# BichenWuUCB/squeezeDet

Measured on NVIDIA H100. Metric: images/sec (1242x375, b=20), higher is better.
Workload: dtype f32 (3xTF32 wgmma, fp32 accumulate)

## Files before the change

include/sqdet_b200.h:

```cpp
#ifndef SQDET_B200_H_
#define SQDET_B200_H_

#include <stdint.h>

#ifdef __cplusplus
extern "C" {
#endif

#define SQDET_OK                 0
#define SQDET_ERR_INVALID_ARG   (-1)
#define SQDET_ERR_CUDA          (-2)
#define SQDET_ERR_UNSUPPORTED   (-3)
#define SQDET_ERR_STATE         (-4)
#define SQDET_ERR_NOT_FOUND     (-5)
#define SQDET_ERR_OVERFLOW      (-6)

#define SQDET_PAD_SAME   0
#define SQDET_PAD_VALID  1

#define SQDET_MATH_FP32_SIMT   0
#define SQDET_MATH_TF32X3_TC   1

typedef struct sqdet_engine sqdet_engine;

// ... 96 lines not shown
                         const int32_t* crops, int order, int rescale, void* stream);
int sqdet_forward_tiles(sqdet_engine* e, int n, int format, const uint8_t* const* planes,
                        const int64_t* pitches, const int32_t* heights, const int32_t* widths,
                        int t, const int32_t* tiles, int order, void* stream);
int sqdet_tile_results_dev(sqdet_engine* e, sqdet_det** dets, int32_t** counts,
                           int32_t* max_dets);
int sqdet_set_box_scale(sqdet_engine* e, const float* xy_scales);
int sqdet_launches_per_forward(sqdet_engine* e);
void* sqdet_engine_stream(sqdet_engine* e);

int sqdet_comm_unique_id(void* id128);
int sqdet_comm_init(sqdet_engine* e, int nranks, int rank, const void* id128);
int sqdet_comm_attach(sqdet_engine* e, void* nccl_comm, int nranks, int rank);
int sqdet_comm_destroy(sqdet_engine* e);
int sqdet_set_gather_in_forward(sqdet_engine* e, int on);
int sqdet_allgather(sqdet_engine* e, void* nccl_comm, void* stream);
int sqdet_gathered_dev(sqdet_engine* e, void** gathered_dev, int64_t* bytes_per_rank,
                       int32_t* nranks);

int sqdet_conv2d(const float* x_dev, const float* w_hwio_dev, const float* bias_dev,
                 const float* scale_dev, const float* shift_dev, float* y_dev,
                 int B, int H, int W, int Cin, int Cout, int size, int stride,
                 int padding, int relu, int y_cstride, int y_coff, int math_mode,
                 void* stream);
int sqdet_conv2d_k_split(const float* x_dev, const float* w_hwio_dev, const float* bias_dev,
                         const float* scale_dev, const float* shift_dev, float* y_dev,
                         int B, int H, int W, int Cin, int Cout, int size, int stride,
                         int padding, int relu, int y_cstride, int y_coff, int math_mode,
                         int k_split, void* stream);
int sqdet_fire(const float* x_dev, const float* w_sq_dev, const float* b_sq_dev,
               const float* w_e1_dev, const float* b_e1_dev, const float* w_e3_dev,
               const float* b_e3_dev, float* y_dev, int B, int H, int W, int Cin, int S,
               int E1, int E3, int math_mode, void* stream);
int sqdet_maxpool_nhwc(const float* x_dev, float* y_dev, int B, int H, int W, int C,
                       int size, int stride, int padding, void* stream);
#define SQDET_PRE_RESIZE_THEN_SUB 0
#define SQDET_PRE_SUB_THEN_RESIZE 1
int sqdet_preprocess_u8(const uint8_t* src_dev, int src_h, int src_w, float* dst_dev,
                        int dst_h, int dst_w, const double* bgr_means, int order,
                        void* stream);
int sqdet_interpret(const float* preds_dev, const float* anchors_f32_dev,
                    float* det_boxes_dev, float* det_probs_dev, int64_t* det_class_dev,
                    int B, int grid_h, int grid_w, int anchors_per_grid, int classes,
                    int image_width, int image_height, float exp_thresh, void* stream);
int sqdet_topk_nms(const float* boxes_dev, const float* probs_dev,
                   const int64_t* cls_dev, int B, int A, int classes, int top_n,
                   float prob_thresh, float nms_thresh, sqdet_det* dets_dev,
                   int32_t* counts_dev, int max_dets, void* stream);
int sqdet_merge_tiles(const float* boxes_dev, const float* probs_dev, const int64_t* cls_dev,
                      int A, int t, const int32_t* tile_frames, const int32_t* tile_xy, int n,
                      int classes, int top_n, float prob_thresh, float nms_thresh,
                      sqdet_det* dets_dev, int32_t* counts_dev, int max_dets, void* stream);
typedef struct sqdet_draw_style {
  int32_t            classes;
  const char* const* class_names;
  const uint8_t*     class_bgr;
  float              plot_prob_thresh;
  float              font_scale;
} sqdet_draw_style;
int sqdet_draw_dets(int n, int format, uint8_t* const* planes, const int64_t* pitches,
                    const int32_t* heights, const int32_t* widths, const int32_t* crops,
                    const sqdet_det* dets_dev, const int32_t* counts_dev, int max_dets,
                    const sqdet_draw_style* style, void* stream);

int64_t sqdet_jpeg_max_bytes(int h, int w);
int64_t sqdet_jpeg_scratch_bytes(int n, const int32_t* heights, const int32_t* widths,
// ... 101 lines not shown
```

squeezedet_b200/_lib.py:

```python
from __future__ import annotations

import ctypes as C
import os

import numpy as np

_HERE = os.path.dirname(os.path.abspath(__file__))
LIB_PATH = os.path.join(_HERE, 'lib', 'libsqdet_b200.so')

OK = 0
PAD_SAME, PAD_VALID = 0, 1
MATH_FP32_SIMT, MATH_TF32X3_TC = 0, 1
IMG_F32, IMG_U8 = 0, 1
_PAD = {'SAME': PAD_SAME, 'VALID': PAD_VALID}


class SqdetError(RuntimeError):
  def __init__(self, code, msg):
    super().__init__('sqdet error %d: %s' % (code, msg))
    self.code = code


class Det(C.Structure):
  _fields_ = [('anchor', C.c_int32), ('cls', C.c_int32), ('prob', C.c_float),
              ('cx', C.c_float), ('cy', C.c_float), ('w', C.c_float),
              ('h', C.c_float)]


DET_DTYPE = np.dtype([('anchor', '<i4'), ('cls', '<i4'), ('prob', '<f4'),
                      ('cx', '<f4'), ('cy', '<f4'), ('w', '<f4'), ('h', '<f4')])
assert DET_DTYPE.itemsize == C.sizeof(Det) == 28


class Config(C.Structure):
  _fields_ = [('batch_size', C.c_int32), ('image_height', C.c_int32),
              ('image_width', C.c_int32), ('classes', C.c_int32),
              ('anchors_per_grid', C.c_int32), ('top_n_detection', C.c_int32),
              ('prob_thresh', C.c_float), ('nms_thresh', C.c_float),
              ('exp_thresh', C.c_float), ('batch_norm_epsilon', C.c_float),
              ('math_mode', C.c_int32), ('max_dets', C.c_int32)]


class DrawStyle(C.Structure):
  _fields_ = [('classes', C.c_int32), ('class_names', C.POINTER(C.c_char_p)),
              ('class_bgr', C.POINTER(C.c_uint8)), ('plot_prob_thresh', C.c_float),
# ... 33 lines not shown
    'sqdet_read_tensor': (_i, [_vp, _i, _fp]),
    'sqdet_num_ops': (_i, [_vp]),
    'sqdet_op_info': (_i, [_vp, _i, C.c_char_p, _i, _i64p, _i64p, _i64p]),
    'sqdet_op_k_split': (_i, [_vp, _i]),
    'sqdet_forward': (_i, [_vp, _fp, _vp]),
    'sqdet_forward_n': (_i, [_vp, _fp, _i, _vp]),
    'sqdet_forward_u8': (_i, [_vp, _vp, _i, _vp]),
    'sqdet_forward_profiled': (_i, [_vp, _fp, _vp, _fp]),
    'sqdet_results_dev': (_i, [_vp, C.POINTER(_vp), C.POINTER(_vp), C.POINTER(_vp),
                               C.POINTER(_vp), C.POINTER(_vp), C.POINTER(C.c_int32)]),
    'sqdet_detect': (_i, [_vp, _fp, _fp, _fp, _fp, _fp, _fp, _vp]),
    'sqdet_set_bgr_means': (_i, [_vp, _vp]),
    'sqdet_submit': (_i, [_vp, _vp, _i, _vp, _vp]),
    'sqdet_wait': (_i, [_vp]),
    'sqdet_submit_frames': (_i, [_vp, _vp, _vp, _vp, _i, _i, _vp, _vp]),
    'sqdet_submit_frames_n': (_i, [_vp, _i, _vp, _vp, _vp, _i, _i, _vp, _vp]),
    'sqdet_forward_frames_u8': (_i, [_vp, _i, _vp, _vp, _vp, _vp, _i, _i, _vp]),
    'sqdet_forward_frames_nv12': (_i, [_vp, _i, _vp, _vp, _vp, _vp, _vp, _vp, _vp, _i, _i, _vp]),
    'sqdet_forward_frames': (_i, [_vp, _i, _i, _vp, _vp, _vp, _vp, _vp, _i, _i, _vp]),
    'sqdet_forward_tiles': (_i, [_vp, _i, _i, _vp, _vp, _vp, _vp, _i, _vp, _i, _vp]),
    'sqdet_tile_results_dev': (_i, [_vp, C.POINTER(_vp), C.POINTER(_vp), C.POINTER(C.c_int32)]),
    'sqdet_set_box_scale': (_i, [_vp, _vp]),
    'sqdet_launches_per_forward': (_i, [_vp]),
    'sqdet_engine_stream': (_vp, [_vp]),
    'sqdet_comm_unique_id': (_i, [_vp]),
    'sqdet_comm_init': (_i, [_vp, _i, _i, _vp]),
    'sqdet_comm_attach': (_i, [_vp, _vp, _i, _i]),
    'sqdet_comm_destroy': (_i, [_vp]),
    'sqdet_set_gather_in_forward': (_i, [_vp, _i]),
    'sqdet_allgather': (_i, [_vp, _vp, _vp]),
    'sqdet_gathered_dev': (_i, [_vp, C.POINTER(_vp), C.POINTER(C.c_int64),
                                C.POINTER(C.c_int32)]),
    'sqdet_fire': (_i, [_fp] * 8 + [_i] * 8 + [_vp]),
    'sqdet_conv2d': (_i, [_fp, _fp, _fp, _fp, _fp, _fp] + [_i] * 12 + [_vp]),
    'sqdet_conv2d_k_split': (_i, [_fp, _fp, _fp, _fp, _fp, _fp] + [_i] * 13 + [_vp]),
    'sqdet_maxpool_nhwc': (_i, [_fp, _fp] + [_i] * 7 + [_vp]),
    'sqdet_preprocess_u8': (_i, [_vp, _i, _i, _fp, _i, _i, _vp, _i, _vp]),
    'sqdet_interpret': (_i, [_fp, _fp, _fp, _fp, _fp] + [_i] * 7 + [_f, _vp]),
    'sqdet_topk_nms': (_i, [_fp, _fp, _fp, _i, _i, _i, _i, _f, _f, _fp, _fp, _i, _vp]),
    'sqdet_merge_tiles': (_i, [_fp, _fp, _fp, _i, _i, _vp, _vp, _i, _i, _i, _f, _f, _fp, _fp, _i,
                               _vp]),
    'sqdet_draw_dets': (_i, [_i, _i, _vp, _vp, _vp, _vp, _vp, _vp, _vp, _i, C.POINTER(DrawStyle),
                             _vp]),
    'sqdet_jpeg_max_bytes': (_i64, [_i, _i]),
    'sqdet_jpeg_scratch_bytes': (_i64, [_i, _vp, _vp, _vp]),
    'sqdet_encode_jpeg': (_i, [_i, _i, _vp, _vp, _vp, _vp, _vp, _i, _vp, _i64, _vp, _vp, _i64, _vp]),
    'sqdet_png_max_bytes': (_i64, [_i, _i]),
    'sqdet_png_scratch_bytes': (_i64, [_i, _vp, _vp, _vp]),
    'sqdet_encode_png': (_i, [_i, _i, _vp, _vp, _vp, _vp, _vp, _vp, _i64, _vp, _vp, _i64, _vp]),
    'sqdet_kitti_eval_scratch_bytes': (_i64, [_i, _i, _i64]),
    'sqdet_kitti_eval': (_i, [_i, _i, _vp, _vp, _i, _vp, _vp, _vp, _i64, _vp, _i64, _vp, _vp]),
    'sqdet_jpeg_parse': (_i, [_vp, _i64, C.POINTER(JpegInfo)]),
    'sqdet_jpeg_decode_staging_bytes': (_i64, [_i, _vp, _vp]),
    'sqdet_jpeg_decode_scratch_bytes': (_i64, [_i, _vp, _vp]),
    'sqdet_decode_jpeg': (_i, [_i, _vp, _vp, _vp, _vp, _vp, _i64, _vp, _i64, _vp, _vp]),
    'sqdet_jpeg_decode_set_subsequence_bits': (_i, [_i]),
    'sqdet_malloc': (_i, [_i, _i64, C.POINTER(_vp)]),
    'sqdet_free': (_i, [_i, _vp]),
    'sqdet_malloc_host': (_i, [_i64, C.POINTER(_vp)]),
    'sqdet_free_host': (_i, [_vp]),
    'sqdet_memcpy_h2d': (_i, [_vp, _vp, _i64, _vp]),
    'sqdet_memcpy_d2h': (_i, [_vp, _vp, _i64, _vp]),
    'sqdet_stream_sync': (_i, [_i, _vp]),
}

_lib = None
# ... 138 lines not shown
```

squeezedet_b200/csrc/conv_tc.cu:

```cuda
#include <cuda.h>
#include <cuda_runtime.h>
#include <stdint.h>
#include <stdlib.h>
#include <string.h>

#include <vector>

#include "common.cuh"
#include "conv_tc.cuh"

namespace sqdet {
namespace {

constexpr int TILE_M = 128;
constexpr int NUM_THREADS = 256;
constexpr int STAGES = 3;
constexpr int MAX_CHUNKS = 32;
constexpr int FT_W = 16, FQ_W = FT_W + 2, FQ_P = 10 * FQ_W;

enum TcMode { TC_ROWS, TC_GATHER, TC_HALO, TC_FIRE };

struct TcChunk {
  int ksize, pad_t, pad_l;
  int nk;
// ... 266 lines not shown
template <int NT, int KC, bool PIPE = true, typename LoadA>
__device__ __forceinline__ void mma_chunk(LoadA load_a, uint32_t bhi, float (&acc)[2][NT / 2],
                                          float (&sum)[NT / 2]) {
  constexpr int KSTEPS = KC / 8;
  uint32_t ahi[2][4], alo[2][4];
  if constexpr (!PIPE) {
#pragma unroll
    for (int ks = 0; ks < KSTEPS; ++ks) {
      load_a(ks, ahi[0], alo[0]);
      mma_step<NT, KC>(acc[0], ahi[0], alo[0], bhi, ks);
      wgmma_wait<0>();
      flush(acc[0], sum, ahi[0], alo[0]);
    }
  } else {
#pragma unroll
    for (int ks = 0; ks < KSTEPS; ++ks) {
      const int cur = ks & 1;
      load_a(ks, ahi[cur], alo[cur]);
      mma_step<NT, KC>(acc[cur], ahi[cur], alo[cur], bhi, ks);
      if (ks > 0) {
        wgmma_wait<1>();
        flush(acc[cur ^ 1], sum, ahi[cur ^ 1], alo[cur ^ 1]);
      }
    }
    constexpr int last = (KSTEPS - 1) & 1;
    wgmma_wait<0>();
    flush(acc[last], sum, ahi[last], alo[last]);
  }
}

struct HaloTile {
  int n, oy0, ox0;
};
__device__ __forceinline__ HaloTile halo_tile(int tiles_w, int tiles_h) {
  const int tx = blockIdx.x % tiles_w, rest = blockIdx.x / tiles_w;
  return {rest / tiles_h, rest % tiles_h * 8, tx * FT_W};
}

__device__ __forceinline__ float finish(const TcParams& p, const TcChunk& ch, int c, float v) {
  if (p.bias) v += p.bias[ch.p_off + c];
  if (p.scale) v = v * p.scale[ch.p_off + c] + p.shift[ch.p_off + c];
  if (p.relu) v = fmaxf(v, 0.f);
  return v;
}

template <typename Value>
__device__ __forceinline__ void store_pair(float* yrow, int c, int ncount, bool pair, Value value) {
  if (pair && c + 1 < ncount) {
    *reinterpret_cast<float2*>(yrow + c) = make_float2(value(c), value(c + 1));
  } else {
    if (c < ncount) yrow[c] = value(c);
    if (c + 1 < ncount) yrow[c + 1] = value(c + 1);
  }
}
__device__ __forceinline__ bool rows_pair_aligned(const TcParams& p, const TcChunk& ch) {
  return ((p.y_cstride | ch.y_off) & 1) == 0 && (reinterpret_cast<uintptr_t>(p.y) & 7) == 0;
}

template <int NT, int KC, int MODE, bool KSPLIT = false>
__global__ void __launch_bounds__(NUM_THREADS, 2)
conv_tc_kernel(const __grid_constant__ TcParams p) {
  static_assert(!KSPLIT || MODE == TC_HALO, "the K split walks halo-mode channel chunks");
  constexpr int NACC = NT / 2;
  constexpr int WST = 2 * NT * KC;
  constexpr uint32_t W_BYTES = WST * 4, TILE_BYTES = TILE_M * KC * 4, HALO_BYTES = FQ_P * KC * 4;
  constexpr int HROWS = halo_rows(KC);
  extern __shared__ __align__(16) uint8_t smem_raw[];
  float* const smem = reinterpret_cast<float*>(smem_raw + ((1024 - (smem_u32(smem_raw) & 1023)) & 1023));
  float* const sa = smem + STAGES * WST;
// ... 133 lines not shown
    cluster_sync();
  } else {
    const bool pair = rows_pair_aligned(p, ch);
#pragma unroll
    for (int h = 0; h < 2; ++h) {
      long long m = m0 + arow0 + 8 * h;
      if (MODE == TC_HALO) {
        const HaloTile tl = halo_tile(p.tiles_w, p.tiles_h);
        const int oy = tl.oy0 + r, ox = tl.ox0 + g + 8 * h;
        if (oy >= p.Ho || ox >= p.Wo) continue;
        m = ((long long)tl.n * p.Ho + oy) * p.Wo + ox;
      } else if (m >= p.M) {
        continue;
      }
      float* yrow = p.y + (size_t)m * p.y_cstride + ch.y_off;
#pragma unroll
      for (int j = 0; j < NT / 8; ++j)
        store_pair(yrow, 8 * j + 2 * t, ch.ncount, pair,
                   [&](int c) { return finish(p, ch, c, sum[4 * j + 2 * h + (c & 1)]); });
    }
  }
}

constexpr int FS = 16;
constexpr int FQ_ROWS = 192;

__host__ __device__ constexpr int fire_stage_floats(int KCI) { return 2 * FS * KCI + FQ_ROWS * KCI; }
constexpr size_t fire_smem_bytes(int KCI) {
  return 1024 + ((size_t)STAGES * fire_stage_floats(KCI) + FQ_ROWS * (FS + 4)) * sizeof(float) +
         2 * STAGES * sizeof(uint64_t);
}

template <int KCI>
__global__ void __launch_bounds__(NUM_THREADS, 2)
fire_tc_kernel(const __grid_constant__ TcParams p) {
  constexpr int QP = FS + 4;
  constexpr int SQW = 2 * FS * KCI;
  constexpr int STAGE = fire_stage_floats(KCI);
  constexpr uint32_t SQW_BYTES = SQW * 4, HALO_BYTES = FQ_P * KCI * 4, EX_BYTES = 2 * 64 * FS * 4;
  static_assert(EX_BYTES <= (SQW + FQ_P * KCI) * 4, "expand tile fits before the zeroed rows");
  static_assert(SQW_BYTES % 1024 == 0 && STAGE * 4 % 1024 == 0, "A tiles keep the swizzle's alignment");
  extern __shared__ __align__(16) uint8_t smem_raw[];
  float* const smem = reinterpret_cast<float*>(smem_raw + ((1024 - (smem_u32(smem_raw) & 1023)) & 1023));
  float* const q = smem + STAGES * STAGE;
  uint64_t* const full = reinterpret_cast<uint64_t*>(q + FQ_ROWS * QP);
  uint64_t* const empty = full + STAGES;

  const int tid = threadIdx.x;
  const int wg = tid >> 7, wq = (tid >> 5) & 3, lane = tid & 31, g = lane >> 2, t = lane & 3;
  const int nks = p.Cin / KCI;
  int total = 0;
#pragma unroll 1
  for (int c = 0; c < p.nchunks; ++c) total += p.chunks[c].nk;
  if (tid == 0) ring_init(full, empty, 1);
  for (int i = tid; i < STAGES * (FQ_ROWS - FQ_P) * KCI; i += NUM_THREADS) {
    const int s = i / ((FQ_ROWS - FQ_P) * KCI);
    smem[s * STAGE + SQW + FQ_P * KCI + i % ((FQ_ROWS - FQ_P) * KCI)] = 0.f;
  }
  __syncthreads();

  auto load_stage = [&](int j) {
    const int s = ring_acquire(empty, j);
    float* const st = smem + s * STAGE;
    if (j < nks) {
      const HaloTile tl = halo_tile(p.tiles_w, p.tiles_h);
      mbar_expect_tx(&full[s], SQW_BYTES + HALO_BYTES);
      tma_load(smem_u32(st + SQW), &p.amap, j * KCI, tl.ox0 - 1, tl.oy0 - 1, tl.n, &full[s]);
      bulk_load(smem_u32(st), p.w + (size_t)j * SQW, SQW_BYTES, &full[s]);
    } else {
      mbar_expect_tx(&full[s], EX_BYTES);
      bulk_load(smem_u32(st), p.w + (size_t)nks * SQW + (size_t)(j - nks) * 2 * 64 * FS, EX_BYTES,
                &full[s]);
    }
  };
  if (tid == 0) {
#pragma unroll 1
    for (int j = 0; j < STAGES - 1 && j < total; ++j) load_stage(j);
  }

  float accq[2][FS / 2], sq[2][FS / 2];
#pragma unroll
  for (int i = 0; i < FS / 2; ++i) accq[0][i] = accq[1][i] = sq[0][i] = sq[1][i] = 0.f;
  const int rb = wq * 16 + g;
  for (int kk = 0; kk < nks; ++kk) {
    if (tid == 0 && kk + STAGES - 1 < total) load_stage(kk + STAGES - 1);
    const float* st = smem + ring_wait_full(full, kk) * STAGE;
    const float* sa = st + SQW;
    if (wg == 0) {
      uint32_t qhi[2][4], qlo[2][4];
#pragma unroll
      for (int j = 0; j < 2 * (KCI / 8); ++j) {
        const int bi = j & 1, ks = j >> 1;
        load_split_swz<KCI>(sa, 128 * bi + rb, ks, t, qhi[bi], qlo[bi]);
        mma_step<FS, KCI>(accq[bi], qhi[bi], qlo[bi], smem_u32(st), ks);
        if (j > 0) {
          wgmma_wait<1>();
          flush(accq[bi ^ 1], sq[bi ^ 1], qhi[bi ^ 1], qlo[bi ^ 1]);
        }
      }
      wgmma_wait<0>();
      flush(accq[1], sq[1], qhi[1], qlo[1]);
    } else {
      mma_chunk<FS, KCI>(
          [&](int ks, uint32_t(&ahi)[4], uint32_t(&alo)[4]) {
            load_split_swz<KCI>(sa, 64 + rb, ks, t, ahi, alo);
// ... 4 lines not shown
  }
  {
    const HaloTile tl = halo_tile(p.tiles_w, p.tiles_h);
#pragma unroll
    for (int bi = 0; bi < 2; ++bi) {
      const int b = wg + 2 * bi;
      if (b >= 3) continue;
#pragma unroll
      for (int h = 0; h < 2; ++h) {
        const int row = b * 64 + wq * 16 + g + 8 * h;
        const int iy = tl.oy0 - 1 + row / FQ_W, ix = tl.ox0 - 1 + row % FQ_W;
        const bool ok = row < FQ_P && iy >= 0 && iy < p.H && ix >= 0 && ix < p.W;
#pragma unroll
        for (int j = 0; j < FS / 8; ++j)
#pragma unroll
          for (int e = 0; e < 2; ++e) {
            const int c = 8 * j + 2 * t + e;
            q[row * QP + c] = ok ? fmaxf(sq[bi][4 * j + 2 * h + e] + p.bias[c], 0.f) : 0.f;
          }
      }
    }
  }
  __syncthreads();

  const int r = wg * 4 + wq;
  float acc[2][32], sum[32];
#pragma unroll
  for (int i = 0; i < 32; ++i) acc[0][i] = acc[1][i] = sum[i] = 0.f;
  int c = 1, kk = 0;
  for (int j = nks; j < total; ++j) {
    if (tid == 0 && j + STAGES - 1 < total) load_stage(j + STAGES - 1);
    const int s = ring_wait_full(full, j);
    const TcChunk& ch = p.chunks[c];
    const int dy = ch.nk == 1 ? 1 : kk / 3, dx = ch.nk == 1 ? 1 : kk % 3;
    const int qr = (r + dy) * FQ_W + g + dx;
    mma_chunk<64, FS>(
        [&](int ks, uint32_t(&ahi)[4], uint32_t(&alo)[4]) {
          load_split(q + qr * QP, q + (qr + 8) * QP, ks, t, ahi, alo);
        },
        smem_u32(smem + s * STAGE), acc, sum);
    ring_release(empty, j);
    if (++kk == ch.nk) {
      const HaloTile tl = halo_tile(p.tiles_w, p.tiles_h);
      const int oy = tl.oy0 + r;
      const size_t prow = ((size_t)tl.n * p.H + oy) * p.W;
      const bool pair = rows_pair_aligned(p, ch);
#pragma unroll
      for (int h = 0; h < 2; ++h) {
        const int ox = tl.ox0 + g + 8 * h;
        if (oy >= p.H || ox >= p.W) continue;
        float* yrow = p.y + (prow + ox) * p.y_cstride + ch.y_off;
#pragma unroll
        for (int jn = 0; jn < 8; ++jn)
          store_pair(yrow, 8 * jn + 2 * t, ch.ncount, pair, [&](int col) {
            return fmaxf(sum[4 * jn + 2 * h + (col & 1)] + p.bias[ch.p_off + col], 0.f);
          });
      }
#pragma unroll
      for (int i = 0; i < 32; ++i) sum[i] = 0.f;
      kk = 0;
      ++c;
    }
  }
}

using TcKernel = void (*)(TcParams);

template <int KC, int MODE>
TcKernel conv_tc_instance(int NT) {
  return NT == 64 ? conv_tc_kernel<64, KC, MODE>
         : NT == 32 ? conv_tc_kernel<32, KC, MODE> : conv_tc_kernel<16, KC, MODE>;
}

TcKernel conv_tc_instance(int NT, int KC, int mode) {
  if (NT == 72) return mode == TC_HALO ? conv_tc_kernel<72, 32, TC_HALO> : conv_tc_kernel<72, 32, TC_ROWS>;
  if (mode == TC_GATHER) return conv_tc_instance<32, TC_GATHER>(NT);
  if (mode == TC_HALO)
    return KC == 32 ? conv_tc_instance<32, TC_HALO>(NT) : conv_tc_instance<16, TC_HALO>(NT);
  return KC == 32 ? conv_tc_instance<32, TC_ROWS>(NT) : conv_tc_instance<16, TC_ROWS>(NT);
}

struct PlanGroup {
  ConvGroup conv;
  int NT, KC, cin, chunk0;
};

}

struct TcImpl {
  TcParams prm{};
  int KC = 0;
  int mode = TC_ROWS;
  TcKernel kernel = nullptr;
  int ksplit = 1;
  size_t smem_bytes = 0;
  std::vector<PlanGroup> groups;
  int cout_total = 0;
  float* d_w = nullptr;
  float* d_bias = nullptr;
  float* d_scale = nullptr;
  float* d_shift = nullptr;
  long long w_floats = 0;
  const float* map_x = nullptr;
  int map_n = 0;
};

static inline float host_rn_tf32(float x) {
  uint32_t u;
  memcpy(&u, &x, 4);
  u = (u + 0x1000u) & 0xFFFFE000u;
  float r;
  memcpy(&r, &u, 4);
  return r;
}

static int pick_nt(const std::vector<ConvGroup>& groups, int KC, bool gather) {
  int best = 0;
  long long best_cost = 0;
  const bool head = !gather && KC == 32 && groups.size() == 1 && groups[0].Cout > 64 &&
                    groups[0].Cout <= 72;
  for (int nt : {72, 64, 32, 16}) {
    if (nt == 72 && !head) continue;
    long long chunks = 0;
    for (const auto& g : groups) chunks += (g.Cout + nt - 1) / nt;
    if (chunks > MAX_CHUNKS) continue;
    const long long cost = chunks * (nt + 32);
    if (!best || cost < best_cost) best = nt, best_cost = cost;
// ... 205 lines not shown
  const bool gather = convs.size() == 1 && Cin == 3 && size == 3 && (stride == 1 || stride == 2) &&
                      convs[0].Cout > 0;
  if (!gather)
    for (const auto& g : convs)
      if (!tc_conv_eligible(Cin, g.Cout, g.ksize, stride, padding)) return 0;
  const Geom gh = tf_geometry(H, size, stride, padding);
  const Geom gw = tf_geometry(W, size, stride, padding);
  if (gh.out <= 0 || gw.out <= 0) return 0;
  const int KC = (gather || Cin % 32 == 0) ? 32 : 16;
  const int NT = pick_nt(convs, KC, gather);
  if (!NT) return 0;
  int mode = gather ? TC_GATHER : TC_ROWS;
  for (const auto& g : convs)
    if (!gather && g.ksize == 3) mode = TC_HALO;
  TcImpl* im = plan->impl = new TcImpl();
  im->KC = KC;
  im->mode = mode;
  im->kernel = conv_tc_instance(NT, KC, mode);
  im->smem_bytes = conv_smem_bytes(NT, KC);
  for (const auto& g : convs) im->groups.push_back({g, NT, KC, Cin, 0});
  int rc = plan_common(im, B, H, W, Cin, gh.out, gw.out, stride, gh.pad_before, gw.pad_before,
                       relu, has_affine, y_cstride);
  if (rc > 0 && NT == 72 && mode == TC_HALO) {
    rc = plan_ksplit(im, k_split);
  } else if (rc > 0 && k_split > 1) {
    rc = fail(SQDET_ERR_INVALID_ARG, "a K split needs a 72-wide 3x3 tensor-core plan");
  }
  if (rc <= 0) tc_conv_release(plan);
  return rc;
}

int tc_conv_k_split(const TcConvPlan& plan) { return plan.impl ? plan.impl->ksplit : 1; }

int tc_fire_plan(TcConvPlan* plan, int B, int H, int W, int Cin, int S, int E1, int E3) {
  plan->impl = nullptr;
  if (Cin % 16 || Cin < 16 || S != FS || E1 <= 0 || E3 <= 0) return 0;
  if ((E1 + 63) / 64 + (E3 + 63) / 64 > 16) return 0;
  const int KCI = Cin % 32 == 0 ? 32 : 16;
  TcImpl* im = plan->impl = new TcImpl();
  im->KC = KCI;
  im->mode = TC_FIRE;
  im->kernel = KCI == 32 ? fire_tc_kernel<32> : fire_tc_kernel<16>;
  im->smem_bytes = fire_smem_bytes(KCI);
  im->groups = {{{1, FS, 0}, FS, KCI, Cin, 0}, {{1, E1, 0}, 64, FS, FS, 0}, {{3, E3, E1}, 64, FS, FS, 0}};
  const int rc = plan_common(im, B, H, W, Cin, H, W, 1, 0, 0, 1, false, E1 + E3);
  if (rc <= 0) tc_conv_release(plan);
  return rc;
}

int tc_conv_pack_weights(TcConvPlan* plan, const std::vector<const float*>& w_hwio,
                         const std::vector<const float*>& bias) {
  TcImpl* im = plan->impl;
  std::vector<float> packed((size_t)im->w_floats, 0.f);
  for (size_t gi = 0; gi < im->groups.size(); ++gi) pack_group(im, im->groups[gi], w_hwio[gi], packed);
  SQ_CUDA(cudaMemcpy(im->d_w, packed.data(), packed.size() * sizeof(float), cudaMemcpyHostToDevice));
  int off = 0;
  for (size_t gi = 0; gi < im->groups.size(); ++gi) {
    const int n = im->groups[gi].conv.Cout;
    if (bias[gi]) SQ_CUDA(cudaMemcpy(im->d_bias + off, bias[gi], sizeof(float) * n, cudaMemcpyHostToDevice));
    off += n;
  }
  return SQDET_OK;
}

int tc_conv_set_affine(TcConvPlan* plan, const float* scale, const float* shift) {
  TcImpl* im = plan->impl;
  if (!im->d_scale) return fail(SQDET_ERR_STATE, "tc conv planned without an affine epilogue");
  SQ_CUDA(cudaMemcpy(im->d_scale, scale, sizeof(float) * im->cout_total, cudaMemcpyHostToDevice));
  SQ_CUDA(cudaMemcpy(im->d_shift, shift, sizeof(float) * im->cout_total, cudaMemcpyHostToDevice));
  return SQDET_OK;
}

int launch_conv_tc(const TcConvPlan& plan, const float* x_dev, float* y_dev, int n,
                   cudaStream_t stream) {
  TcImpl* im = plan.impl;
  if (n < 1 || n > im->prm.B) return fail(SQDET_ERR_INVALID_ARG, "launch_conv_tc: image count outside [1, B]");
  const int rc = update_maps(im, x_dev, n);
  if (rc) return rc;
  TcParams prm = im->prm;
  prm.x = x_dev;
  prm.y = y_dev;
  prm.B = n;
  prm.M = (long long)n * prm.Ho * prm.Wo;
  const dim3 grid((unsigned)grid_blocks(im, n), im->mode == TC_FIRE ? 1u : (unsigned)prm.nchunks);
  if (im->ksplit > 1) {
    const ClusterLaunch l(grid, im->smem_bytes, im->ksplit, stream);
    SQ_CUDA(cudaLaunchKernelEx(&l.cfg, im->kernel, prm));
  } else {
    im->kernel<<<grid, NUM_THREADS, im->smem_bytes, stream>>>(prm);
  }
  SQ_CHECK_LAUNCH(im->mode == TC_FIRE ? "fire_tc_kernel" : "conv_tc_kernel");
  return SQDET_OK;
}

void tc_conv_release(TcConvPlan* plan) {
  TcImpl* im = plan->impl;
  if (!im) return;
  cudaFree(im->d_w);
  cudaFree(im->d_bias);
  cudaFree(im->d_scale);
  cudaFree(im->d_shift);
  delete im;
  plan->impl = nullptr;
}

int tc_conv_oneshot(TcConvPlan* plan, const std::vector<const float*>& w_hwio_dev,
                    const std::vector<const float*>& bias_dev, const float* scale_dev,
                    const float* shift_dev, const float* x_dev, float* y_dev, cudaStream_t stream) {
  TcImpl* im = plan->impl;
  if (!im) return 1;
  const size_t ng = im->groups.size();
  std::vector<std::vector<float>> w(ng), b(ng);
  std::vector<float> sc, sh;
  std::vector<const float*> w_host(ng), b_host(ng);
  cudaError_t ce = cudaSuccess;
  auto download = [&ce](std::vector<float>& dst, const float* src, size_t n) {
// ... 23 lines not shown
```

squeezedet_b200/csrc/conv_tc.cuh:

```cuda
#pragma once
#include <cuda_runtime.h>
#include <stdint.h>

#include <vector>

namespace sqdet {

struct ConvGroup {
  int ksize, Cout, y_off;
};

struct TcImpl;

struct TcConvPlan {
  TcImpl* impl = nullptr;
};

bool tc_conv_eligible(int Cin, int Cout, int size, int stride, int padding);

int tc_conv_plan(TcConvPlan* plan, int B, int H, int W, int Cin, const std::vector<ConvGroup>& convs,
                 int stride, int padding, int relu, bool has_affine, int y_cstride, int k_split = 0);
int tc_conv_k_split(const TcConvPlan& plan);
int tc_fire_plan(TcConvPlan* plan, int B, int H, int W, int Cin, int S, int E1, int E3);
int tc_conv_pack_weights(TcConvPlan* plan, const std::vector<const float*>& w_hwio,
                         const std::vector<const float*>& bias);
int tc_conv_set_affine(TcConvPlan* plan, const float* scale, const float* shift);
int launch_conv_tc(const TcConvPlan& plan, const float* x_dev, float* y_dev, int n,
                   cudaStream_t stream);
void tc_conv_release(TcConvPlan* plan);

int tc_conv_oneshot(TcConvPlan* plan, const std::vector<const float*>& w_hwio_dev,
                    const std::vector<const float*>& bias_dev, const float* scale_dev,
                    const float* shift_dev, const float* x_dev, float* y_dev, cudaStream_t stream);

}
```

squeezedet_b200/csrc/engine.cu:

```cuda
#include <cuda_runtime.h>
#include <dlfcn.h>
#include <math.h>
#include <stdio.h>
#include <stdlib.h>
#include <string.h>

#include <functional>
#include <map>
#include <memory>
#include <string>
#include <vector>

#include "common.cuh"
#include "conv_tc.cuh"

namespace sqdet {

static thread_local std::string g_last_error;

void set_error(const std::string& msg) { g_last_error = msg; }

int fail(int code, const std::string& msg) {
  g_last_error = msg;
  return code;
// ... 1492 lines not shown
                         int y_cstride, int y_coff, int math_mode, int k_split, void* stream) {
  if (!x_dev || !w_hwio_dev || !y_dev) return fail(SQDET_ERR_INVALID_ARG, "sqdet_conv2d: null pointer");
  if (k_split < 0 || k_split > 4) return fail(SQDET_ERR_INVALID_ARG, "sqdet_conv2d: k_split outside [0, 4]");
  if (k_split > 1 && math_mode != SQDET_MATH_TF32X3_TC)
    return fail(SQDET_ERR_INVALID_ARG, "sqdet_conv2d: a K split needs SQDET_MATH_TF32X3_TC");
  if (padding != SQDET_PAD_SAME && padding != SQDET_PAD_VALID)
    return fail(SQDET_ERR_INVALID_ARG, "sqdet_conv2d: padding must be SAME(0) or VALID(1)");
  if (int rc = check_conv_epilogue("sqdet_conv2d", scale_dev, shift_dev, Cout, y_cstride, y_coff))
    return rc;
  if (math_mode != SQDET_MATH_FP32_SIMT && math_mode != SQDET_MATH_TF32X3_TC)
    return fail(SQDET_ERR_INVALID_ARG, "sqdet_conv2d: unknown math_mode");
  if (math_mode == SQDET_MATH_TF32X3_TC) {
    TcConvPlan plan;
    int rc = tc_conv_plan(&plan, B, H, W, Cin, {{size, Cout, y_coff}}, stride, padding, relu,
                          scale_dev != nullptr, y_cstride, k_split);
    if (rc >= 0)
      rc = tc_conv_oneshot(&plan, {w_hwio_dev}, {bias_dev}, scale_dev, shift_dev, x_dev, y_dev,
                           (cudaStream_t)stream);
    if (rc == 1 && k_split > 1)
      return fail(SQDET_ERR_INVALID_ARG, "sqdet_conv2d: a K split needs a shape the tensor-core path takes");
    if (rc != 1) return rc;
  }
  ConvArgs a;
  a.x = x_dev; a.w = w_hwio_dev; a.bias = bias_dev; a.scale = scale_dev; a.shift = shift_dev;
  a.y = y_dev; a.B = B; a.H = H; a.W = W; a.Cin = Cin; a.Cout = Cout; a.size = size;
  a.stride = stride; a.padding = padding; a.relu = relu; a.y_cstride = y_cstride; a.y_coff = y_coff;
  return launch_conv_simt(a, (cudaStream_t)stream);
}

int sqdet_fire(const float* x_dev, const float* w_sq_dev, const float* b_sq_dev,
               const float* w_e1_dev, const float* b_e1_dev, const float* w_e3_dev,
               const float* b_e3_dev, float* y_dev, int B, int H, int W, int Cin, int S, int E1,
               int E3, int math_mode, void* stream_v) {
  if (!x_dev || !w_sq_dev || !b_sq_dev || !w_e1_dev || !b_e1_dev || !w_e3_dev || !b_e3_dev || !y_dev)
    return fail(SQDET_ERR_INVALID_ARG, "sqdet_fire: null pointer");
  if (B <= 0 || H <= 0 || W <= 0 || Cin <= 0 || S <= 0 || E1 <= 0 || E3 <= 0)
    return fail(SQDET_ERR_INVALID_ARG, "sqdet_fire: non-positive dimension");
  if (math_mode != SQDET_MATH_FP32_SIMT && math_mode != SQDET_MATH_TF32X3_TC)
    return fail(SQDET_ERR_INVALID_ARG, "sqdet_fire: unknown math_mode");
  cudaStream_t stream = (cudaStream_t)stream_v;
  if (math_mode == SQDET_MATH_TF32X3_TC) {
    TcConvPlan plan;
    int rc = tc_fire_plan(&plan, B, H, W, Cin, S, E1, E3);
    if (rc >= 0)
      rc = tc_conv_oneshot(&plan, {w_sq_dev, w_e1_dev, w_e3_dev}, {b_sq_dev, b_e1_dev, b_e3_dev},
                           nullptr, nullptr, x_dev, y_dev, stream);
    if (rc != 1) return rc;
  }
  float* q = nullptr;
  SQ_CUDA(cudaMalloc(&q, sizeof(float) * (size_t)B * H * W * S));
  int rc = sqdet_conv2d(x_dev, w_sq_dev, b_sq_dev, nullptr, nullptr, q, B, H, W, Cin, S, 1, 1,
                        SQDET_PAD_SAME, 1, S, 0, math_mode, stream_v);
  if (!rc)
    rc = sqdet_conv2d(q, w_e1_dev, b_e1_dev, nullptr, nullptr, y_dev, B, H, W, S, E1, 1, 1,
                      SQDET_PAD_SAME, 1, E1 + E3, 0, math_mode, stream_v);
  if (!rc)
    rc = sqdet_conv2d(q, w_e3_dev, b_e3_dev, nullptr, nullptr, y_dev, B, H, W, S, E3, 3, 1,
                      SQDET_PAD_SAME, 1, E1 + E3, E1, math_mode, stream_v);
  cudaError_t ce = cudaStreamSynchronize(stream);
  cudaFree(q);
  if (rc) return rc;
  if (ce != cudaSuccess) return cuda_fail(ce, "sqdet_fire sync");
  return SQDET_OK;
}

int sqdet_maxpool_nhwc(const float* x_dev, float* y_dev, int B, int H, int W, int C, int size,
                       int stride, int padding, void* stream) {
  if (!x_dev || !y_dev) return fail(SQDET_ERR_INVALID_ARG, "sqdet_maxpool_nhwc: null pointer");
  if (padding != SQDET_PAD_SAME && padding != SQDET_PAD_VALID)
    return fail(SQDET_ERR_INVALID_ARG, "sqdet_maxpool_nhwc: padding must be SAME(0) or VALID(1)");
  return launch_maxpool(x_dev, y_dev, B, H, W, C, size, stride, padding, (cudaStream_t)stream);
}

int sqdet_preprocess_u8(const uint8_t* src_dev, int src_h, int src_w, float* dst_dev, int dst_h,
                        int dst_w, const double* bgr_means, int order, void* stream) {
  if (!src_dev || !dst_dev || !bgr_means)
    return fail(SQDET_ERR_INVALID_ARG, "sqdet_preprocess_u8: null pointer");
  if (order != SQDET_PRE_RESIZE_THEN_SUB && order != SQDET_PRE_SUB_THEN_RESIZE)
    return fail(SQDET_ERR_INVALID_ARG, "sqdet_preprocess_u8: order must be 0 (demo) or 1 (eval)");
// ... 76 lines not shown
```

Baseline: 4842.

## Add resident-weight persistent fire kernel and multi-tap expand weight staging

```diff
diff --git a/include/sqdet_b200.h b/include/sqdet_b200.h
--- a/include/sqdet_b200.h
+++ b/include/sqdet_b200.h
@@ -152,6 +152,14 @@
                const float* w_e1_dev, const float* b_e1_dev, const float* w_e3_dev,
                const float* b_e3_dev, float* y_dev, int B, int H, int W, int Cin, int S,
                int E1, int E3, int math_mode, void* stream);
+#define SQDET_FIRE_AUTO 0
+#define SQDET_FIRE_STREAMING 1
+#define SQDET_FIRE_RESIDENT 2
+int sqdet_fire_variant(const float* x_dev, const float* w_sq_dev, const float* b_sq_dev,
+                       const float* w_e1_dev, const float* b_e1_dev, const float* w_e3_dev,
+                       const float* b_e3_dev, float* y_dev, int B, int H, int W, int Cin,
+                       int S, int E1, int E3, int math_mode, int variant, int max_ctas,
+                       void* stream);
 int sqdet_maxpool_nhwc(const float* x_dev, float* y_dev, int B, int H, int W, int C,
                        int size, int stride, int padding, void* stream);
 #define SQDET_PRE_RESIZE_THEN_SUB 0
diff --git a/squeezedet_b200/_lib.py b/squeezedet_b200/_lib.py
--- a/squeezedet_b200/_lib.py
+++ b/squeezedet_b200/_lib.py
@@ -11,6 +11,7 @@
 OK = 0
 PAD_SAME, PAD_VALID = 0, 1
 MATH_FP32_SIMT, MATH_TF32X3_TC = 0, 1
+FIRE_AUTO, FIRE_STREAMING, FIRE_RESIDENT = 0, 1, 2
 IMG_F32, IMG_U8 = 0, 1
 _PAD = {'SAME': PAD_SAME, 'VALID': PAD_VALID}
 
@@ -110,6 +111,7 @@
     'sqdet_gathered_dev': (_i, [_vp, C.POINTER(_vp), C.POINTER(C.c_int64),
                                 C.POINTER(C.c_int32)]),
     'sqdet_fire': (_i, [_fp] * 8 + [_i] * 8 + [_vp]),
+    'sqdet_fire_variant': (_i, [_fp] * 8 + [_i] * 10 + [_vp]),
     'sqdet_conv2d': (_i, [_fp, _fp, _fp, _fp, _fp, _fp] + [_i] * 12 + [_vp]),
     'sqdet_conv2d_k_split': (_i, [_fp, _fp, _fp, _fp, _fp, _fp] + [_i] * 13 + [_vp]),
     'sqdet_maxpool_nhwc': (_i, [_fp, _fp] + [_i] * 7 + [_vp]),
diff --git a/squeezedet_b200/csrc/conv_tc.cu b/squeezedet_b200/csrc/conv_tc.cu
--- a/squeezedet_b200/csrc/conv_tc.cu
+++ b/squeezedet_b200/csrc/conv_tc.cu
@@ -322,9 +322,12 @@
 struct HaloTile {
   int n, oy0, ox0;
 };
+__device__ __forceinline__ HaloTile halo_tile(unsigned tile, int tiles_w, int tiles_h) {
+  const int tx = tile % tiles_w, rest = tile / tiles_w;
+  return {rest / tiles_h, rest % tiles_h * 8, tx * FT_W};
+}
 __device__ __forceinline__ HaloTile halo_tile(int tiles_w, int tiles_h) {
-  const int tx = blockIdx.x % tiles_w, rest = blockIdx.x / tiles_w;
-  return {rest / tiles_h, rest % tiles_h * 8, tx * FT_W};
+  return halo_tile(blockIdx.x, tiles_w, tiles_h);
 }
 
 __device__ __forceinline__ float finish(const TcParams& p, const TcChunk& ch, int c, float v) {
@@ -524,13 +527,102 @@
 }
 
 template <int KCI>
+__device__ __forceinline__ void squeeze_chunk(const float* sa, uint32_t bw, int wg, int rb, int t,
+                                              float (&accq)[2][FS / 2], float (&sq)[2][FS / 2]) {
+  if (wg == 0) {
+    uint32_t qhi[2][4], qlo[2][4];
+#pragma unroll
+    for (int j = 0; j < 2 * (KCI / 8); ++j) {
+      const int bi = j & 1, ks = j >> 1;
+      load_split_swz<KCI>(sa, 128 * bi + rb, ks, t, qhi[bi], qlo[bi]);
+      mma_step<FS, KCI>(accq[bi], qhi[bi], qlo[bi], bw, ks);
+      if (j > 0) {
+        wgmma_wait<1>();
+        flush(accq[bi ^ 1], sq[bi ^ 1], qhi[bi ^ 1], qlo[bi ^ 1]);
+      }
+    }
+    wgmma_wait<0>();
+    flush(accq[1], sq[1], qhi[1], qlo[1]);
+  } else {
+    mma_chunk<FS, KCI>(
+        [&](int ks, uint32_t(&ahi)[4], uint32_t(&alo)[4]) {
+          load_split_swz<KCI>(sa, 64 + rb, ks, t, ahi, alo);
+        },
+        bw, accq, sq[0]);
+  }
+}
+
+__device__ __forceinline__ void store_q(const TcParams& p, const HaloTile& tl, float* q, int wg, int wq,
+                                        int g, int t, const float (&sq)[2][FS / 2]) {
+  constexpr int QP = FS + 4;
+#pragma unroll
+  for (int bi = 0; bi < 2; ++bi) {
+    const int b = wg + 2 * bi;
+    if (b >= 3) continue;
+#pragma unroll
+    for (int h = 0; h < 2; ++h) {
+      const int row = b * 64 + wq * 16 + g + 8 * h;
+      const int iy = tl.oy0 - 1 + row / FQ_W, ix = tl.ox0 - 1 + row % FQ_W;
+      const bool ok = row < FQ_P && iy >= 0 && iy < p.H && ix >= 0 && ix < p.W;
+#pragma unroll
+      for (int j = 0; j < FS / 8; ++j)
+#pragma unroll
+        for (int e = 0; e < 2; ++e) {
+          const int c = 8 * j + 2 * t + e;
+          q[row * QP + c] = ok ? fmaxf(sq[bi][4 * j + 2 * h + e] + p.bias[c], 0.f) : 0.f;
+        }
+    }
+  }
+}
+
+__device__ __forceinline__ void store_expand(const TcParams& p, const TcChunk& ch, const HaloTile& tl,
+                                             int r, int g, int t, const float (&sum)[32]) {
+  const int oy = tl.oy0 + r;
+  const size_t prow = ((size_t)tl.n * p.H + oy) * p.W;
+  const bool pair = rows_pair_aligned(p, ch);
+#pragma unroll
+  for (int h = 0; h < 2; ++h) {
+    const int ox = tl.ox0 + g + 8 * h;
+    if (oy >= p.H || ox >= p.W) continue;
+    float* yrow = p.y + (prow + ox) * p.y_cstride + ch.y_off;
+#pragma unroll
+    for (int jn = 0; jn < 8; ++jn)
+      store_pair(yrow, 8 * jn + 2 * t, ch.ncount, pair, [&](int col) {
+        return fmaxf(sum[4 * jn + 2 * h + (col & 1)] + p.bias[ch.p_off + col], 0.f);
+      });
+  }
+}
+
+template <int TAPS>
+__device__ __forceinline__ void expand_chunk(const float* q, int qr0, int t, uint32_t w0,
+                                             float (&acc)[2][32], float (&sum)[32]) {
+  constexpr int QP = FS + 4, NSTEPS = 2 * TAPS;
+  constexpr uint32_t TAP_BYTES = 2 * 64 * FS * 4;
+  uint32_t ahi[2][4], alo[2][4];
+#pragma unroll
+  for (int i = 0; i < NSTEPS; ++i) {
+    const int cur = i & 1, tap = i / 2, ks = i & 1;
+    const int qr = qr0 + tap / 3 * FQ_W + tap % 3;
+    load_split(q + qr * QP, q + (qr + 8) * QP, ks, t, ahi[cur], alo[cur]);
+    mma_step<64, FS>(acc[cur], ahi[cur], alo[cur], w0 + tap * TAP_BYTES, ks);
+    if (i > 0) {
+      wgmma_wait<1>();
+      flush(acc[cur ^ 1], sum, ahi[cur ^ 1], alo[cur ^ 1]);
+    }
+  }
+  wgmma_wait<0>();
+  flush(acc[1], sum, ahi[1], alo[1]);
+}
+
+template <int KCI>
 __global__ void __launch_bounds__(NUM_THREADS, 2)
 fire_tc_kernel(const __grid_constant__ TcParams p) {
   constexpr int QP = FS + 4;
   constexpr int SQW = 2 * FS * KCI;
   constexpr int STAGE = fire_stage_floats(KCI);
   constexpr uint32_t SQW_BYTES = SQW * 4, HALO_BYTES = FQ_P * KCI * 4, EX_BYTES = 2 * 64 * FS * 4;
-  static_assert(EX_BYTES <= (SQW + FQ_P * KCI) * 4, "expand tile fits before the zeroed rows");
+  constexpr int EX_TAPS = KCI == 32 ? 3 : 1;
+  static_assert(EX_TAPS * EX_BYTES <= (SQW + FQ_P * KCI) * 4, "expand tiles fit before the zeroed rows");
   static_assert(SQW_BYTES % 1024 == 0 && STAGE * 4 % 1024 == 0, "A tiles keep the swizzle's alignment");
   extern __shared__ __align__(16) uint8_t smem_raw[];
   float* const smem = reinterpret_cast<float*>(smem_raw + ((1024 - (smem_u32(smem_raw) & 1023)) & 1023));
@@ -541,9 +633,9 @@
   const int tid = threadIdx.x;
   const int wg = tid >> 7, wq = (tid >> 5) & 3, lane = tid & 31, g = lane >> 2, t = lane & 3;
   const int nks = p.Cin / KCI;
-  int total = 0;
+  int total = nks;
 #pragma unroll 1
-  for (int c = 0; c < p.nchunks; ++c) total += p.chunks[c].nk;
+  for (int c = 1; c < p.nchunks; ++c) total += (p.chunks[c].nk + EX_TAPS - 1) / EX_TAPS;
   if (tid == 0) ring_init(full, empty, 1);
   for (int i = tid; i < STAGES * (FQ_ROWS - FQ_P) * KCI; i += NUM_THREADS) {
     const int s = i / ((FQ_ROWS - FQ_P) * KCI);
@@ -551,6 +643,7 @@
   }
   __syncthreads();
 
+  int lc = 1, ltap = 0;
   auto load_stage = [&](int j) {
     const int s = ring_acquire(empty, j);
     float* const st = smem + s * STAGE;
@@ -560,9 +653,12 @@
       tma_load(smem_u32(st + SQW), &p.amap, j * KCI, tl.ox0 - 1, tl.oy0 - 1, tl.n, &full[s]);
       bulk_load(smem_u32(st), p.w + (size_t)j * SQW, SQW_BYTES, &full[s]);
     } else {
-      mbar_expect_tx(&full[s], EX_BYTES);
-      bulk_load(smem_u32(st), p.w + (size_t)nks * SQW + (size_t)(j - nks) * 2 * 64 * FS, EX_BYTES,
-                &full[s]);
+      const TcChunk& ch = p.chunks[lc];
+      const uint32_t bytes = (ch.nk - ltap < EX_TAPS ? ch.nk - ltap : EX_TAPS) * EX_BYTES;
+      mbar_expect_tx(&full[s], bytes);
+      bulk_load(smem_u32(st), p.w + ch.w_off + (size_t)ltap * 2 * 64 * FS, bytes, &full[s]);
+      ltap += EX_TAPS;
+      if (ltap >= ch.nk) ltap = 0, ++lc;
     }
   };
   if (tid == 0) {
@@ -633,34 +729,122 @@
     if (tid == 0 && j + STAGES - 1 < total) load_stage(j + STAGES - 1);
     const int s = ring_wait_full(full, j);
     const TcChunk& ch = p.chunks[c];
-    const int dy = ch.nk == 1 ? 1 : kk / 3, dx = ch.nk == 1 ? 1 : kk % 3;
-    const int qr = (r + dy) * FQ_W + g + dx;
-    mma_chunk<64, FS>(
-        [&](int ks, uint32_t(&ahi)[4], uint32_t(&alo)[4]) {
-          load_split(q + qr * QP, q + (qr + 8) * QP, ks, t, ahi, alo);
-        },
-        smem_u32(smem + s * STAGE), acc, sum);
+    const uint32_t w0 = smem_u32(smem + s * STAGE);
+    if (EX_TAPS == 1 || ch.nk == 1) {
+      const int tap = ch.nk == 1 ? 4 : kk;
+      expand_chunk<1>(q, (r + tap / 3) * FQ_W + g + tap % 3, t, w0, acc, sum);
+      ++kk;
+    } else {
+      expand_chunk<EX_TAPS>(q, (r + kk / 3) * FQ_W + g + kk % 3, t, w0, acc, sum);
+      kk += EX_TAPS;
+    }
     ring_release(empty, j);
-    if (++kk == ch.nk) {
-      const HaloTile tl = halo_tile(p.tiles_w, p.tiles_h);
-      const int oy = tl.oy0 + r;
-      const size_t prow = ((size_t)tl.n * p.H + oy) * p.W;
-      const bool pair = rows_pair_aligned(p, ch);
-#pragma unroll
-      for (int h = 0; h < 2; ++h) {
-        const int ox = tl.ox0 + g + 8 * h;
-        if (oy >= p.H || ox >= p.W) continue;
-        float* yrow = p.y + (prow + ox) * p.y_cstride + ch.y_off;
-#pragma unroll
-        for (int jn = 0; jn < 8; ++jn)
-          store_pair(yrow, 8 * jn + 2 * t, ch.ncount, pair, [&](int col) {
-            return fmaxf(sum[4 * jn + 2 * h + (col & 1)] + p.bias[ch.p_off + col], 0.f);
-          });
-      }
+    if (kk == ch.nk) {
+      store_expand(p, ch, halo_tile(p.tiles_w, p.tiles_h), r, g, t, sum);
 #pragma unroll
       for (int i = 0; i < 32; ++i) sum[i] = 0.f;
       kk = 0;
       ++c;
+    }
+  }
+}
+
+__host__ __device__ constexpr size_t fire_res_fixed_bytes(int KCI) {
+  return ((size_t)STAGES * FQ_ROWS * KCI + 2 * FQ_ROWS * (FS + 4)) * sizeof(float) + 8 * sizeof(uint64_t);
+}
+constexpr size_t fire_res_smem_bytes(int KCI, long long w_floats) {
+  return 1024 + fire_res_fixed_bytes(KCI) + (size_t)w_floats * sizeof(float);
+}
+
+template <int KCI>
+__global__ void __launch_bounds__(NUM_THREADS, 1)
+fire_res_kernel(const __grid_constant__ TcParams p, long long w_floats) {
+  constexpr int QP = FS + 4;
+  constexpr int SQW = 2 * FS * KCI;
+  constexpr int STAGE = FQ_ROWS * KCI;
+  constexpr uint32_t HALO_BYTES = FQ_P * KCI * 4;
+  static_assert(STAGE * 4 % 1024 == 0, "A tiles keep the swizzle's alignment");
+  extern __shared__ __align__(16) uint8_t smem_raw[];
+  float* const smem = reinterpret_cast<float*>(smem_raw + ((1024 - (smem_u32(smem_raw) & 1023)) & 1023));
+  float* const qbuf = smem + STAGES * STAGE;
+  uint64_t* const full = reinterpret_cast<uint64_t*>(qbuf + 2 * FQ_ROWS * QP);
+  uint64_t* const empty = full + STAGES;
+  uint64_t* const wbar = empty + STAGES;
+  float* const wres = reinterpret_cast<float*>(full + 8);
+
+  const int tid = threadIdx.x;
+  const int wg = tid >> 7, wq = (tid >> 5) & 3, lane = tid & 31, g = lane >> 2, t = lane & 3;
+  const int nks = p.Cin / KCI;
+  const int ntiles = p.B * p.tiles_h * p.tiles_w;
+  const int mine = (ntiles - (int)blockIdx.x + (int)gridDim.x - 1) / (int)gridDim.x;
+  const int total = mine * nks;
+  if (tid == 0) {
+    ring_init(full, empty, 1);
+    mbar_init(wbar, 1);
+    mbar_init_fence();
+    const uint32_t bytes = (uint32_t)(w_floats * 4);
+    mbar_expect_tx(wbar, bytes);
+    constexpr uint32_t PIECE = 32768;
+    for (uint32_t off = 0; off < bytes; off += PIECE)
+      bulk_load(smem_u32(wres) + off, reinterpret_cast<const uint8_t*>(p.w) + off,
+                bytes - off < PIECE ? bytes - off : PIECE, wbar);
+  }
+  for (int i = tid; i < STAGES * (FQ_ROWS - FQ_P) * KCI; i += NUM_THREADS) {
+    const int s = i / ((FQ_ROWS - FQ_P) * KCI);
+    smem[s * STAGE + FQ_P * KCI + i % ((FQ_ROWS - FQ_P) * KCI)] = 0.f;
+  }
+  __syncthreads();
+
+  int issued = 0;
+  auto issue = [&](int limit) {
+    for (; issued < limit && issued < total; ++issued) {
+      const int j = issued, s = ring_acquire(empty, j);
+      const HaloTile tl = halo_tile(blockIdx.x + (unsigned)(j / nks) * gridDim.x, p.tiles_w, p.tiles_h);
+      mbar_expect_tx(&full[s], HALO_BYTES);
+      tma_load(smem_u32(smem + s * STAGE), &p.amap, j % nks * KCI, tl.ox0 - 1, tl.oy0 - 1, tl.n, &full[s]);
+    }
+  };
+  if (tid == 0) issue(STAGES);
+  mbar_wait(wbar, 0);
+
+  const int rb = wq * 16 + g;
+  const int r = wg * 4 + wq;
+  const uint32_t w_u32 = smem_u32(wres);
+#pragma unroll 1
+  for (int i = 0; i < mine; ++i) {
+    const HaloTile tl = halo_tile(blockIdx.x + (unsigned)i * gridDim.x, p.tiles_w, p.tiles_h);
+    float* const q = qbuf + (i & 1) * FQ_ROWS * QP;
+    float accq[2][FS / 2], sq[2][FS / 2];
+#pragma unroll
+    for (int k = 0; k < FS / 2; ++k) accq[0][k] = accq[1][k] = sq[0][k] = sq[1][k] = 0.f;
+#pragma unroll 1
+    for (int kk = 0; kk < nks; ++kk) {
+      const int j = i * nks + kk;
+      if (tid == 0) issue(j + STAGES);
+      const int s = ring_wait_full(full, j);
+      squeeze_chunk<KCI>(smem + s * STAGE, w_u32 + kk * SQW * 4, wg, rb, t, accq, sq);
+      ring_release(empty, j);
+    }
+    store_q(p, tl, q, wg, wq, g, t, sq);
+    __syncthreads();
+    if (tid == 0) issue((i + 1) * nks + STAGES);
+
+    float acc[2][32], sum[32];
+#pragma unroll
+    for (int k = 0; k < 32; ++k) acc[0][k] = acc[1][k] = sum[k] = 0.f;
+    const int qr0 = r * FQ_W + g;
+#pragma unroll 1
+    for (int c = 1; c < p.nchunks; ++c) {
+      const TcChunk& ch = p.chunks[c];
+      const uint32_t w0 = w_u32 + (uint32_t)ch.w_off * 4;
+      if (ch.nk == 9) {
+        expand_chunk<9>(q, qr0, t, w0, acc, sum);
+      } else {
+        expand_chunk<1>(q, qr0 + FQ_W + 1, t, w0, acc, sum);
+      }
+      store_expand(p, ch, tl, r, g, t, sum);
+#pragma unroll
+      for (int k = 0; k < 32; ++k) sum[k] = 0.f;
     }
   }
 }
@@ -694,6 +878,8 @@
   int mode = TC_ROWS;
   TcKernel kernel = nullptr;
   int ksplit = 1;
+  void (*res_kernel)(TcParams, long long) = nullptr;
+  int res_ctas = 0;
   size_t smem_bytes = 0;
   std::vector<PlanGroup> groups;
   int cout_total = 0;
@@ -965,8 +1151,27 @@
 
 int tc_conv_k_split(const TcConvPlan& plan) { return plan.impl ? plan.impl->ksplit : 1; }
 
-int tc_fire_plan(TcConvPlan* plan, int B, int H, int W, int Cin, int S, int E1, int E3) {
+static int plan_fire_resident(TcImpl* im, int variant, int max_ctas) {
+  if (variant != TC_FIRE_RESIDENT) return 1;
+  int dev = 0, optin = 0, sms = 0;
+  SQ_CUDA(cudaGetDevice(&dev));
+  SQ_CUDA(cudaDeviceGetAttribute(&optin, cudaDevAttrMaxSharedMemoryPerBlockOptin, dev));
+  SQ_CUDA(cudaDeviceGetAttribute(&sms, cudaDevAttrMultiProcessorCount, dev));
+  const size_t smem = fire_res_smem_bytes(im->KC, im->w_floats);
+  if (smem > (size_t)optin)
+    return fail(SQDET_ERR_INVALID_ARG, "the fire's weights do not fit the resident-weight kernel");
+  im->res_kernel = im->KC == 32 ? fire_res_kernel<32> : fire_res_kernel<16>;
+  SQ_CUDA(cudaFuncSetAttribute(im->res_kernel, cudaFuncAttributeMaxDynamicSharedMemorySize, (int)smem));
+  im->smem_bytes = smem;
+  im->res_ctas = max_ctas > 0 ? max_ctas : sms;
+  return 1;
+}
+
+int tc_fire_plan(TcConvPlan* plan, int B, int H, int W, int Cin, int S, int E1, int E3, int variant,
+                 int max_ctas) {
   plan->impl = nullptr;
+  if (variant < TC_FIRE_AUTO || variant > TC_FIRE_RESIDENT || max_ctas < 0)
+    return fail(SQDET_ERR_INVALID_ARG, "tc_fire_plan: unknown variant or negative CTA cap");
   if (Cin % 16 || Cin < 16 || S != FS || E1 <= 0 || E3 <= 0) return 0;
   if ((E1 + 63) / 64 + (E3 + 63) / 64 > 16) return 0;
   const int KCI = Cin % 32 == 0 ? 32 : 16;
@@ -976,7 +1181,8 @@
   im->kernel = KCI == 32 ? fire_tc_kernel<32> : fire_tc_kernel<16>;
   im->smem_bytes = fire_smem_bytes(KCI);
   im->groups = {{{1, FS, 0}, FS, KCI, Cin, 0}, {{1, E1, 0}, 64, FS, FS, 0}, {{3, E3, E1}, 64, FS, FS, 0}};
-  const int rc = plan_common(im, B, H, W, Cin, H, W, 1, 0, 0, 1, false, E1 + E3);
+  int rc = plan_common(im, B, H, W, Cin, H, W, 1, 0, 0, 1, false, E1 + E3);
+  if (rc > 0) rc = plan_fire_resident(im, variant, max_ctas);
   if (rc <= 0) tc_conv_release(plan);
   return rc;
 }
@@ -1015,6 +1221,13 @@
   prm.y = y_dev;
   prm.B = n;
   prm.M = (long long)n * prm.Ho * prm.Wo;
+  if (im->res_kernel) {
+    const long long tiles = grid_blocks(im, n);
+    const unsigned ctas = (unsigned)(tiles < im->res_ctas ? tiles : im->res_ctas);
+    im->res_kernel<<<ctas, NUM_THREADS, im->smem_bytes, stream>>>(prm, im->w_floats);
+    SQ_CHECK_LAUNCH("fire_res_kernel");
+    return SQDET_OK;
+  }
   const dim3 grid((unsigned)grid_blocks(im, n), im->mode == TC_FIRE ? 1u : (unsigned)prm.nchunks);
   if (im->ksplit > 1) {
     const ClusterLaunch l(grid, im->smem_bytes, im->ksplit, stream);
diff --git a/squeezedet_b200/csrc/conv_tc.cuh b/squeezedet_b200/csrc/conv_tc.cuh
--- a/squeezedet_b200/csrc/conv_tc.cuh
+++ b/squeezedet_b200/csrc/conv_tc.cuh
@@ -21,7 +21,9 @@
 int tc_conv_plan(TcConvPlan* plan, int B, int H, int W, int Cin, const std::vector<ConvGroup>& convs,
                  int stride, int padding, int relu, bool has_affine, int y_cstride, int k_split = 0);
 int tc_conv_k_split(const TcConvPlan& plan);
-int tc_fire_plan(TcConvPlan* plan, int B, int H, int W, int Cin, int S, int E1, int E3);
+enum { TC_FIRE_AUTO = 0, TC_FIRE_STREAMING = 1, TC_FIRE_RESIDENT = 2 };
+int tc_fire_plan(TcConvPlan* plan, int B, int H, int W, int Cin, int S, int E1, int E3,
+                 int variant = TC_FIRE_AUTO, int max_ctas = 0);
 int tc_conv_pack_weights(TcConvPlan* plan, const std::vector<const float*>& w_hwio,
                          const std::vector<const float*>& bias);
 int tc_conv_set_affine(TcConvPlan* plan, const float* scale, const float* shift);
diff --git a/squeezedet_b200/csrc/engine.cu b/squeezedet_b200/csrc/engine.cu
--- a/squeezedet_b200/csrc/engine.cu
+++ b/squeezedet_b200/csrc/engine.cu
@@ -1548,6 +1548,23 @@
                const float* w_e1_dev, const float* b_e1_dev, const float* w_e3_dev,
                const float* b_e3_dev, float* y_dev, int B, int H, int W, int Cin, int S, int E1,
                int E3, int math_mode, void* stream_v) {
+  return sqdet_fire_variant(x_dev, w_sq_dev, b_sq_dev, w_e1_dev, b_e1_dev, w_e3_dev, b_e3_dev, y_dev,
+                            B, H, W, Cin, S, E1, E3, math_mode, SQDET_FIRE_AUTO, 0, stream_v);
+}
+
+static_assert(SQDET_FIRE_AUTO == TC_FIRE_AUTO && SQDET_FIRE_STREAMING == TC_FIRE_STREAMING &&
+                  SQDET_FIRE_RESIDENT == TC_FIRE_RESIDENT,
+              "sqdet_fire_variant passes its variant to tc_fire_plan");
+
+int sqdet_fire_variant(const float* x_dev, const float* w_sq_dev, const float* b_sq_dev,
+                       const float* w_e1_dev, const float* b_e1_dev, const float* w_e3_dev,
+                       const float* b_e3_dev, float* y_dev, int B, int H, int W, int Cin, int S,
+                       int E1, int E3, int math_mode, int variant, int max_ctas, void* stream_v) {
+  if (variant < SQDET_FIRE_AUTO || variant > SQDET_FIRE_RESIDENT)
+    return fail(SQDET_ERR_INVALID_ARG, "sqdet_fire: variant outside [0, 2]");
+  if (max_ctas < 0) return fail(SQDET_ERR_INVALID_ARG, "sqdet_fire: negative CTA cap");
+  if (variant != SQDET_FIRE_AUTO && math_mode != SQDET_MATH_TF32X3_TC)
+    return fail(SQDET_ERR_INVALID_ARG, "sqdet_fire: a forced variant needs SQDET_MATH_TF32X3_TC");
   if (!x_dev || !w_sq_dev || !b_sq_dev || !w_e1_dev || !b_e1_dev || !w_e3_dev || !b_e3_dev || !y_dev)
     return fail(SQDET_ERR_INVALID_ARG, "sqdet_fire: null pointer");
   if (B <= 0 || H <= 0 || W <= 0 || Cin <= 0 || S <= 0 || E1 <= 0 || E3 <= 0)
@@ -1557,10 +1574,12 @@
   cudaStream_t stream = (cudaStream_t)stream_v;
   if (math_mode == SQDET_MATH_TF32X3_TC) {
     TcConvPlan plan;
-    int rc = tc_fire_plan(&plan, B, H, W, Cin, S, E1, E3);
+    int rc = tc_fire_plan(&plan, B, H, W, Cin, S, E1, E3, variant, max_ctas);
     if (rc >= 0)
       rc = tc_conv_oneshot(&plan, {w_sq_dev, w_e1_dev, w_e3_dev}, {b_sq_dev, b_e1_dev, b_e3_dev},
                            nullptr, nullptr, x_dev, y_dev, stream);
+    if (rc == 1 && variant != SQDET_FIRE_AUTO)
+      return fail(SQDET_ERR_INVALID_ARG, "sqdet_fire: a forced variant needs a shape the one-kernel fire takes");
     if (rc != 1) return rc;
   }
   float* q = nullptr;
```

Measured after the change: 4858, median of 6. Within noise of the previous version (+0.3%).
